# XDzzzzzZyq/b-pinn-kalman-filter

Measured on AMD Instinct MI355X. Metric: PC-sampler score-net evals/s (NCSN++ 128x128x1, EM + Langevin), higher is better.
Workload: dtype f32; 1 GPU; configs[2]: NCSN++ 128x128x1 PC sampler, VP-SDE N=1000, euler_maruyama + langevin (snr 0.075), global batch 64 = 64/GPU x 1; model=ncsnpp (62.69M params), global_batch=64, per_gpu_batch=64, parallelism=dp1 (batch-sharded, RCCL), hip_graph=True, pc_graph_allreduce=False

## Files before the change

b-pinn-kalman-filter_amd/csrc/conv_winograd.hip:

```cpp
#include "bpk_common.h"

#include <algorithm>
#include <cstdlib>
#include <type_traits>

namespace {

using f4 = __attribute__((ext_vector_type(4))) float;

constexpr int kTR = 4, kTC = 8;
constexpr int kM = kTR * kTC;
constexpr int kPR = 2 * kTR + 2;
constexpr int kPC = 2 * kTC + 2;
constexpr int kPCp = 24;
constexpr int kCK = 8;
constexpr int kOutRows = 2 * kTR, kOutCols = 2 * kTC;

__device__ inline void wino_filter_range(const float* __restrict__ w, float* __restrict__ U,
                                         int Cin, int Cout, int CoutP, int ft, int64_t first,
                                         int64_t stride) {
  const int64_t total = (int64_t)Cin * CoutP;
  for (int64_t i = first; i < total; i += stride) {
    const int co = (int)(i % CoutP);
    const int ci = (int)(i / CoutP);
    if (co >= Cout) {
      f4* u = reinterpret_cast<f4*>(U + ((int64_t)ci * CoutP + co) * 16);
#pragma unroll
      for (int r = 0; r < 4; ++r) u[r] = f4{0.f, 0.f, 0.f, 0.f};
      continue;
    }
    const float* g = ft ? w + ((int64_t)ci * Cout + co) * 9 : w + ((int64_t)co * Cin + ci) * 9;
    auto gv = [&](int k) { return ft ? g[8 - k] : g[k]; };
    float t[4][3];
#pragma unroll
    for (int c = 0; c < 3; ++c) {
      const float g0 = gv(c), g1 = gv(3 + c), g2 = gv(6 + c);
      t[0][c] = g0;
      t[1][c] = 0.5f * (g0 + g1 + g2);
      t[2][c] = 0.5f * (g0 - g1 + g2);
      t[3][c] = g2;
    }
    float* u = U + ((int64_t)ci * CoutP + co) * 16;
#pragma unroll
    for (int r = 0; r < 4; ++r) {
      const float a0 = t[r][0], a1 = t[r][1], a2 = t[r][2];
      u[4 * r + 0] = a0;
      u[4 * r + 1] = 0.5f * (a0 + a1 + a2);
      u[4 * r + 2] = 0.5f * (a0 - a1 + a2);
      u[4 * r + 3] = a2;
    }
  }
}

__global__ __launch_bounds__(256) void wino_filter_kernel(const float* __restrict__ w,
                                                          float* __restrict__ U, int Cin,
                                                          int Cout, int CoutP, int ft) {
  wino_filter_range(w, U, Cin, Cout, CoutP, ft, (int64_t)blockIdx.x * blockDim.x + threadIdx.x,
                    (int64_t)gridDim.x * blockDim.x);
}

__global__ __launch_bounds__(256) void wino_filter_batch_kernel(const int64_t* __restrict__ jobs) {
  const int64_t* jb = jobs + 6 * (int64_t)blockIdx.y;
  wino_filter_range(reinterpret_cast<const float*>(jb[0]), reinterpret_cast<float*>(jb[1]),
                    (int)jb[2], (int)jb[3], (int)jb[4], (int)jb[5],
                    (int64_t)blockIdx.x * blockDim.x + threadIdx.x,
                    (int64_t)gridDim.x * blockDim.x);
}

struct WinoGeo {
  int N, Cin, Cout, H, W;
  int regions_x, regions_y, cout_blocks;
  float div;
  int C1;
  int CoutS;
  int up;
  int ksplit;
  int pair;
};

constexpr int kVS = 20;
constexpr int kOS = kOutRows * kOutCols + 4;
constexpr int kPatchPerThread = (kCK * kPR * kPC + 255) / 256;
constexpr int kPreMaxCin = 1024;


__device__ inline float silu_f(float z) { return z * __builtin_amdgcn_rcpf(1.f + __expf(-z)); }

__device__ inline unsigned udivmod(unsigned a, unsigned d, unsigned& r) {
  if ((d & (d - 1)) == 0) {
    r = a & (d - 1);
    return a >> __builtin_ctz(d);
  }
  const unsigned q = a / d;
  r = a - q * d;
  return q;
}

__device__ inline float div_rn(float a, float b, float r) {
  const float q = a * r;
// ... 845 lines not shown
      }
    }
    if (!PAIR && stats) {
      merge_stats(lm, lm2, __shfl_xor(lm, 16, 64), __shfl_xor(lm2, 16, 64), 32.f);
      merge_stats(lm, lm2, __shfl_xor(lm, 32, 64), __shfl_xor(lm2, 32, 64), 64.f);
      if (kq == 0) {
        const int R = g.regions_x * g.regions_y;
        const int region = (oy0 / kOutRows) * g.regions_x + ox0 / kOutCols;
        stats[((int64_t)n * g.CoutS + co) * R + region] = make_float2(lm, lm2);
      }
    }
  }
  WINO_TS(5);
}

template <bool PRE, bool PAIR = false>
__global__ __launch_bounds__(512, 1) void wino_f23_k16_kernel(
    const float* __restrict__ x, const float* __restrict__ U, const float* __restrict__ bias,
    const float* __restrict__ skip, const float2* __restrict__ pre, float* __restrict__ y,
    float2* __restrict__ stats, WinoGeo g, int xcd_remap, const float* __restrict__ x2,
    unsigned items) {
  const unsigned G = gridDim.x, w = blockIdx.x;
  unsigned first = w, stride = G, end = items;
  if (xcd_remap) {
    const unsigned xc = w & 7u, q = items >> 3, r = items & 7u;
    const unsigned start = xc * q + min(xc, r);
    first = start + (w >> 3);
    stride = G >> 3;
    end = start + q + (xc < r ? 1u : 0u);
  }
  for (unsigned b = first; b < end; b += stride) {
    if (b != first) __syncthreads();
    k16_item<PRE, PAIR>(b, x, U, bias, skip, pre, y, stats, g, x2);
  }
}

__global__ __launch_bounds__(256) void wino_splitk_reduce_kernel(
    const float* __restrict__ part, int S, const float* __restrict__ bias,
    const float* __restrict__ skip, float* __restrict__ y, float2* __restrict__ stats,
    WinoGeo g) {
  const int lane = threadIdx.x & 63;
  const int q = threadIdx.x;
  unsigned b = blockIdx.x, reg, cg;
  const unsigned R = (unsigned)(g.regions_x * g.regions_y);
  unsigned r = udivmod(b, R, reg);
  int n = (int)udivmod(r, (unsigned)(g.CoutS / 8), cg);
  const int co = (int)cg * 8 + (q >> 5);
  const int rem = q & 31;
  const int row = rem >> 2;
  int c4 = rem & 3;
  if (g.pair) {
    n = 2 * n + (c4 >> 1);
    c4 &= 1;
  }
  const int oy0 = (int)(reg / g.regions_x) * kOutRows, ox0 = (int)(reg % g.regions_x) * kOutCols;
  const int64_t plane = (int64_t)g.H * g.W;
  const int64_t slab = (int64_t)g.N * g.CoutS * plane;
  const int64_t o = ((int64_t)n * g.CoutS + co) * plane + (int64_t)(oy0 + row) * g.W + ox0 + 4 * c4;
  f4 v = *reinterpret_cast<const f4*>(&part[o]);
  for (int s = 1; s < S; ++s) v += *reinterpret_cast<const f4*>(&part[s * slab + o]);
  const float bv = bias ? bias[co] : 0.f;
  v += f4{bv, bv, bv, bv};
  if (skip) {
    const f4 sk = *reinterpret_cast<const f4*>(&skip[o]);
    const float rdiv = 1.f / g.div;
#pragma unroll
// ... 265 lines not shown
                       U, nullptr, nullptr, kpre, workspace, nullptr, gk, remap, x2, (unsigned)items);
  BPK_LAUNCH_CHECK("conv3x3_wino_splitk");
  const int64_t rblocks = (int64_t)N * (Cout / 8) * gk.regions_x * gk.regions_y;
  BPK_REQUIRE(Cout % 8 == 0 && rblocks < (1LL << 31), "conv3x3_wino_splitk: reduce grid");
  hipLaunchKernelGGL(wino_splitk_reduce_kernel, dim3((unsigned)rblocks), dim3(256), 0, st,
                     workspace, S, bias, skip, y, reinterpret_cast<float2*>(stats), gk);
  BPK_LAUNCH_CHECK("conv3x3_wino_splitk_reduce");
  return BPK_OK;
}

extern "C" int bpk_conv3x3_wino_up2_supported(int N, int Cin, int Cout, int H, int W) {
  return bpk_conv3x3_wino_supported(N, Cin, Cout, H, W) && Cin % 16 == 0 &&
         cout_padded(Cout) % 128 == 0;
}

extern "C" int bpk_conv3x3_wino_up2_f32(const float* x, const float* U, const float* bias,
                                        float* y, int N, int Cin, int Cout, int H, int W,
                                        void* stream) {
  BPK_REQUIRE(bpk_conv3x3_wino_up2_supported(N, Cin, Cout, H, W),
              "conv3x3_wino_up2: unsupported shape N=%d Cin=%d Cout=%d H=%d W=%d (need Cin %% 16, "
              "Cout %% 128, H %% 8, W %% 16 == 0)", N, Cin, Cout, H, W);
  const int CoutP = cout_padded(Cout);
  WinoGeo gk{N, Cin, CoutP, H, W, W / kOutCols, H / kOutRows, CoutP / 128, 1.0f, Cin, Cout, 1};
  const int64_t items = (int64_t)N * gk.regions_x * gk.regions_y * gk.cout_blocks;
  BPK_REQUIRE(items < (1LL << 31), "conv3x3_wino_up2: grid too large");
  const unsigned kg = k16_grid(items);
  hipLaunchKernelGGL((wino_f23_k16_kernel<false>), dim3(kg), dim3(512), 0,
                     bpk::as_stream(stream), x, U, bias, nullptr, nullptr, y, nullptr, gk,
                     (kg % 8 == 0) ? 1 : 0, nullptr, (unsigned)items);
  BPK_LAUNCH_CHECK("conv3x3_wino_up2");
  return BPK_OK;
}

extern "C" int bpk_conv3x3_wino_pre_f32(const float* x, const float* pre, const float* U,
                                        const float* bias, const float* skip, float div, float* y,
                                        int N, int Cin, int Cout, int H, int W, void* stream) {
  return bpk_conv3x3_wino_ex_f32(x, nullptr, Cin, pre, U, bias, skip, div, y, nullptr, N, Cin,
                                 Cout, H, W, stream);
}

extern "C" int bpk_conv3x3_wino_residual_f32(const float* x, const float* U, const float* bias,
                                             const float* skip, float div, float* y, int N,
                                             int Cin, int Cout, int H, int W, void* stream) {
  return bpk_conv3x3_wino_pre_f32(x, nullptr, U, bias, skip, div, y, N, Cin, Cout, H, W, stream);
}

extern "C" int bpk_conv3x3_wino_f32(const float* x, const float* U, const float* bias, float* y,
                                    int N, int Cin, int Cout, int H, int W, void* stream) {
  return bpk_conv3x3_wino_pre_f32(x, nullptr, U, bias, nullptr, 1.0f, y, N, Cin, Cout, H, W,
                                  stream);
}

#ifdef WINO_TIMING
extern "C" int bpk_wino_timing_read(long long* ts, unsigned* cu, int n) {
  if (n > (int)kTsMax) n = (int)kTsMax;
  if (hipMemcpyFromSymbol(ts, HIP_SYMBOL(g_wino_ts), sizeof(long long) * 8 * n) != hipSuccess) return -1;
  if (hipMemcpyFromSymbol(cu, HIP_SYMBOL(g_wino_cu), sizeof(unsigned) * n) != hipSuccess) return -1;
  return n;
}
#endif
```

b-pinn-kalman-filter_amd/op/conv.py:

```python
from __future__ import annotations

import contextlib
import functools
import os

import torch
import torch.nn.functional as F
from torch.autograd.function import once_differentiable

from . import flops
from ._lib import check, lib, require_hip, stream_ptr, mark_inputs, want_grad


def _shape_ok(x, weight):
    return (x.dtype == torch.float32 and weight.dtype == torch.float32 and x.dim() == 4
            and tuple(weight.shape[2:]) == (3, 3) and x.is_cuda and weight.shape[1] == x.shape[1])


def wino_supported(x, weight):
    if not _shape_ok(x, weight):
        return False
    N, C, H, W = x.shape
    return bool(lib.bpk_conv3x3_wino_supported(N, C, weight.shape[0], H, W))


def wino_pair_supported(x, weight):
    if not _shape_ok(x, weight):
        return False
    N, C, H, W = x.shape
    return bool(lib.bpk_conv3x3_wino_pair_supported(N, C, weight.shape[0], H, W))


def small_supported(x, weight):
    if not _shape_ok(x, weight):
        return False
    N, C, H, W = x.shape
    return bool(lib.bpk_conv3x3_small_supported(N, C, weight.shape[0], H, W))


def supported(x, weight):
    return small_supported(x, weight) or wino_supported(x, weight)


_STATIC_FILTERS = None


@contextlib.contextmanager
def static_filters(registry: list):
    global _STATIC_FILTERS
    prev, _STATIC_FILTERS = _STATIC_FILTERS, registry
    try:
        yield registry
    finally:
        _STATIC_FILTERS = prev


def _transform_into(weight, U, ft):
    w = weight.detach().contiguous()
    Cout, Cin = (w.shape[1], w.shape[0]) if ft else (w.shape[0], w.shape[1])
    fn = lib.bpk_conv3x3_wino_filter_ft_f32 if ft else lib.bpk_conv3x3_wino_filter_f32
    check(fn(w.data_ptr(), U.data_ptr(), Cin, Cout, stream_ptr(w.device)), "conv3x3 filter")


def refresh_filters(registry: list):
    for i, (weight, U, ft, ver) in enumerate(registry):
        if weight._version != ver:
            _transform_into(weight, U, ft)
            registry[i] = (weight, U, ft, weight._version)


_FILTER_BATCH = None


class FilterBatch:

    def __init__(self, module):
        jobs, self.map, self.params = [], {}, []
        dev = None
        for m in module.modules():
            if not (isinstance(m, torch.nn.Conv2d) and m.kernel_size == (3, 3)
                    and m.stride == (1, 1) and m.padding == (1, 1) and m.dilation == (1, 1)
                    and m.groups == 1):
                continue
            w = m.weight
            if not (w.is_cuda and w.dtype == torch.float32 and w.is_contiguous()):
                continue
            dev = w.device
            self.params.append(w)
            for ft in (False, True):
                Cout, Cin = (w.shape[1], w.shape[0]) if ft else (w.shape[0], w.shape[1])
                key = (w.data_ptr(), ft)
                if Cin % 8 or Cout % 16 or key in self.map:
                    continue
                CoutP = lib.bpk_conv3x3_wino_filter_bytes(Cin, Cout) // (16 * 4 * Cin)
                U = torch.empty((Cin, CoutP, 16), dtype=torch.float32, device=w.device)
                self.map[key] = (tuple(w.shape), U)
                jobs.append([w.data_ptr(), U.data_ptr(), Cin, Cout, CoutP, int(ft)])
        self.n = len(jobs)
        self.max_elems = max((j[2] * j[4] for j in jobs), default=0)
        self.jobs = torch.tensor(jobs, dtype=torch.int64).to(dev) if jobs else None
        self.ptrs = [w.data_ptr() for w in self.params]
# ... 6 lines not shown
            check(lib.bpk_conv3x3_wino_filter_batch_f32(
                self.jobs.data_ptr(), self.n, self.max_elems, stream_ptr(self.jobs.device)),
                "conv3x3 filter batch")

    @contextlib.contextmanager
    def active(self):
        global _FILTER_BATCH
        prev, _FILTER_BATCH = _FILTER_BATCH, self.map
        try:
            yield self
        finally:
            _FILTER_BATCH = prev


def filter_batch_for(module) -> "FilterBatch":
    fb = getattr(module, "_bpk_filter_batch", None)
    if fb is None or not fb.valid_for(module):
        fb = FilterBatch(module)
        object.__setattr__(module, "_bpk_filter_batch", fb)
    return fb


@contextlib.contextmanager
def batched_filters(module, enabled=True):
    if not enabled:
        yield None
        return
    fb = filter_batch_for(module)
    fb.refresh()
    with fb.active():
        yield fb


def filter_transform(weight, ft=False):
    fbm = _FILTER_BATCH
    if fbm is not None and weight.is_contiguous():
        e = fbm.get((weight.data_ptr(), bool(ft)))
        if e is not None and e[0] == tuple(weight.shape):
            return e[1]
    attr = "_bpk_wino_u_ft" if ft else "_bpk_wino_u"
    capturing = torch.cuda.is_current_stream_capturing()
    cached = getattr(weight, attr, None)
    if capturing and _STATIC_FILTERS is not None and cached is not None \
            and cached[0] == weight._version:
        if not any(e[1] is cached[1] for e in _STATIC_FILTERS):
            _STATIC_FILTERS.append((weight, cached[1], ft, weight._version))
        return cached[1]
    if capturing:
        cached = None
    if cached is not None and cached[0] == weight._version:
        return cached[1]
    w = weight.detach().contiguous()
    Cout, Cin = (w.shape[1], w.shape[0]) if ft else (w.shape[0], w.shape[1])
    CoutP = lib.bpk_conv3x3_wino_filter_bytes(Cin, Cout) // (16 * 4 * Cin)
    U = torch.empty((Cin, CoutP, 16), dtype=torch.float32, device=w.device)
    fn = lib.bpk_conv3x3_wino_filter_ft_f32 if ft else lib.bpk_conv3x3_wino_filter_f32
    check(fn(w.data_ptr(), U.data_ptr(), Cin, Cout, stream_ptr(w.device)), "conv3x3 filter")
    if not capturing:
        setattr(weight, attr, (weight._version, U))
    return U


GN_PART_COUNT = 128


def gn_partials(t):
    p = getattr(t, "_bpk_gn_part", None)
    if p is None or p[3] != t._version:
        return None
    return p[:3]


def attach_gn_partials(t, part, R, cnt=GN_PART_COUNT):
    t._bpk_gn_part = (part, R, cnt, t._version)
    return t


def ensure_gn_partials(t):
    p = gn_partials(t)
    if p is not None:
        return p
    if (t.dim() != 4 or not t.is_cuda or t.dtype != torch.float32 or not t.is_contiguous()
            or (t.shape[2] * t.shape[3]) % GN_PART_COUNT != 0):
        return None
    N, C, H, W = t.shape
    R = H * W // GN_PART_COUNT
    part = torch.empty((N, C, R, 2), dtype=torch.float32, device=t.device)
    check(lib.bpk_group_norm_chunk_partials_f32(t.data_ptr(), part.data_ptr(), N, C, H * W,
                                                stream_ptr(t.device)), "gn_partials")
    attach_gn_partials(t, part, R)
    return part, R, GN_PART_COUNT


def conv3x3_fwd_raw(x, weight, bias=None, skip=None, div=1.0, pre=None, stats=False, x2=None,
                    ft=False):
    x = x.contiguous()
    N, C1, H, W = x.shape
    C = C1 if x2 is None else C1 + x2.shape[1]
    if x2 is not None:
        x2 = x2.contiguous()
        if x2.shape[0] != N or tuple(x2.shape[2:]) != (H, W) or C1 % 8:
            raise RuntimeError(f"conv3x3: second source {tuple(x2.shape)} vs {tuple(x.shape)}")
    Cout = weight.shape[1] if ft else weight.shape[0]
    U = filter_transform(weight, ft)
    y = torch.empty((N, Cout, H, W), dtype=x.dtype, device=x.device)
    b = None if bias is None else bias.detach().contiguous()
    sk = None if skip is None else skip.detach().contiguous()
    if sk is not None and sk.shape != y.shape:
        raise RuntimeError(f"conv3x3: skip {tuple(sk.shape)} != output {tuple(y.shape)}")
    pr = None if pre is None else pre.contiguous()
    if pr is not None and tuple(pr.shape) != (N, C, 2):
        raise RuntimeError(f"conv3x3: pre must be [N, Cin, 2], got {tuple(pr.shape)}")
    part = None
    if stats:
        R = (H // 8) * (W // 16)
        part = torch.empty((N, Cout, R, 2), dtype=torch.float32, device=x.device)
    nws = lib.bpk_conv3x3_wino_splitk_bytes(N, C, C1 if x2 is not None else C, Cout, H, W)
    ws = torch.empty(nws // 4, dtype=torch.float32, device=x.device) if nws > 0 else None
    check(lib.bpk_conv3x3_wino_splitk_f32(
        x.data_ptr(), None if x2 is None else x2.data_ptr(), C1,
        None if pr is None else pr.data_ptr(), U.data_ptr(),
        None if b is None else b.data_ptr(), None if sk is None else sk.data_ptr(), float(div),
        y.data_ptr(), None if part is None else part.data_ptr(),
        None if ws is None else ws.data_ptr(), N, C, Cout, H, W,
        stream_ptr(x.device)), "conv3x3_wino")
    flops.wino3x3("wino_dgrad" if ft else "wino_fwd", N, C, Cout, H, W)
    if part is not None:
        attach_gn_partials(y, part, R)
    return y


_WGRAD = True


def wgrad_supported(x, weight):
    if not _WGRAD:
        return False
    if x.dtype != torch.float32 or x.dim() != 4 or not x.is_cuda:
        return False
    N, C, H, W = x.shape
    cout = weight[0] if isinstance(weight, (tuple, list, torch.Size)) else weight.shape[0]
    return bool(lib.bpk_conv3x3_wino_wgrad_supported(N, C, cout, H, W))


def conv3x3_wgrad_raw(x, gy, wshape, bias_grad=False, pre=None):
    x = x.detach().contiguous()
    gy = gy.detach().contiguous()
    N, C, H, W = x.shape
    Cout = wshape[0]
    if tuple(gy.shape) != (N, Cout, H, W) or tuple(wshape[1:]) != (C, 3, 3):
        raise RuntimeError(f"conv3x3_wgrad: x {tuple(x.shape)}, gy {tuple(gy.shape)}, "
                           f"w {tuple(wshape)}")
    nbytes = lib.bpk_conv3x3_wino_wgrad_workspace_bytes(N, C, Cout, H, W)
    ws = torch.empty(nbytes // 4, dtype=torch.float32, device=x.device)
    dw = torch.empty((Cout, C, 3, 3), dtype=torch.float32, device=x.device)
    db = torch.empty((Cout,), dtype=torch.float32, device=x.device) if bias_grad else None
    pr = None if pre is None else pre.detach().contiguous()
    if pr is not None and tuple(pr.shape) != (N, C, 2):
        raise RuntimeError(f"conv3x3_wgrad: pre must be [N, Cin, 2], got {tuple(pr.shape)}")
# ... 756 lines not shown
    __slots__ = ("g",)

    def __init__(self):
        self.g = None


def gn_silu_conv3x3_ad(x, num_groups, gamma, beta, eps, weight, bias=None, skip=None, div=1.0,
                       bias_nc=None, give=None, take=None, fanout=False):
    require_hip(x, weight, bias, skip, bias_nc, what="gn_silu_conv3x3_ad")
    if not gn_silu_conv3x3_ad_supported(x, weight):
        return None
    if skip is not None and tuple(skip.shape) != (x.shape[0], weight.shape[0]) + tuple(x.shape[2:]):
        return None
    stats = bool(wino_supported(x, weight))
    return _GNSiLUConv3x3.apply(x, bias_nc, gamma, beta, weight, bias, skip, num_groups,
                                float(eps), float(div), stats, give, take, bool(fanout))


def up2_supported(x, weight):
    if not (_WINO_UP2 and x.is_cuda and x.dtype == torch.float32 and x.dim() == 4
            and weight.dtype == torch.float32 and tuple(weight.shape[1:]) == (x.shape[1], 3, 3)):
        return False
    N, C, H, W = x.shape
    return bool(lib.bpk_conv3x3_wino_up2_supported(N, C, weight.shape[0], 2 * H, 2 * W))


_WINO_UP2 = True


def _up2_raw(x, weight, bias):
    x = x.detach().contiguous()
    N, C, H, W = x.shape
    Cout = weight.shape[0]
    U = filter_transform(weight, False)
    y = torch.empty((N, Cout, 2 * H, 2 * W), dtype=x.dtype, device=x.device)
    b = None if bias is None else bias.detach().contiguous()
    check(lib.bpk_conv3x3_wino_up2_f32(x.data_ptr(), U.data_ptr(),
                                       None if b is None else b.data_ptr(), y.data_ptr(),
                                       N, C, Cout, 2 * H, 2 * W, stream_ptr(x.device)),
          "conv3x3_wino_up2")
    flops.wino3x3("wino_fwd", N, C, Cout, 2 * H, 2 * W)
    return y


class _Sum2x2(torch.autograd.Function):

    @staticmethod
    def forward(ctx, g):
        N, C, H2, W2 = g.shape
        if g.is_cuda and g.dtype == torch.float32:
            g = g.contiguous()
            y = torch.empty((N, C, H2 // 2, W2 // 2), device=g.device, dtype=g.dtype)
            check(lib.bpk_sum2x2_f32(g.data_ptr(), y.data_ptr(), N * C, H2 // 2, W2 // 2,
                                     stream_ptr(g.device)), "sum2x2")
            return y
        return g.reshape(N, C, H2 // 2, 2, W2 // 2, 2).sum((3, 5))

    @staticmethod
    def backward(ctx, gg):
        return F.interpolate(gg, scale_factor=2, mode="nearest")


def _sum2x2(g):
    if g.shape[2] % 2 or g.shape[3] % 2:
        raise RuntimeError(f"_sum2x2: even spatial sizes expected, got {tuple(g.shape)}")
    return _Sum2x2.apply(g)


class _ConvUp2(torch.autograd.Function):

    @staticmethod
    def forward(ctx, x, w, b):
        mark_inputs(ctx, x, w, b)
        ctx.save_for_backward(x, w)
# ... 335 lines not shown
```

b-pinn-kalman-filter_amd/op/flops.py:

```python
from __future__ import annotations

import contextlib

_ACTIVE: list = []


class Tally:
    def __init__(self):
        self.executed = 0.0
        self.direct = 0.0
        self.by_kind: dict = {}
        self.aten = 0.0

    def add(self, kind, executed, direct):
        self.executed += executed
        self.direct += direct
        e, d, n = self.by_kind.get(kind, (0.0, 0.0, 0))
        self.by_kind[kind] = (e + executed, d + direct, n + 1)

    @property
    def total_executed(self):
        return self.executed + self.aten

    @property
    def total_direct(self):
        return self.direct + self.aten

    def summary(self):
        return {"executed_flop": self.total_executed, "direct_flop": self.total_direct,
                "aten_flop": self.aten,
                "native": {k: {"executed": e, "direct": d, "launches": n}
                           for k, (e, d, n) in sorted(self.by_kind.items())}}


def add(kind, executed, direct=None):
    if _ACTIVE:
        for t in _ACTIVE:
            t.add(kind, float(executed), float(executed if direct is None else direct))


def wino3x3(kind, N, C, Cout, H, W):
    if _ACTIVE:
        add(kind, 32.0 * N * C * Cout * ((H + 1) // 2) * ((W + 1) // 2), 18.0 * N * C * Cout * H * W)


def _aten_mode():
    from torch.utils._python_dispatch import TorchDispatchMode
    from torch.utils.flop_counter import flop_registry

    class AtenFlops(TorchDispatchMode):
        total = 0

        def __torch_dispatch__(self, func, types, args=(), kwargs=None):
            kwargs = kwargs or {}
            out = func(*args, **kwargs)
            f = flop_registry.get(func._overloadpacket)
            if f is not None:
                self.total += f(*args, **kwargs, out_val=out)
            return out

    return AtenFlops()


@contextlib.contextmanager
def counting(aten=True):
    t = Tally()
    _ACTIVE.append(t)
    mode = _aten_mode() if aten else contextlib.nullcontext()
    try:
        with mode:
            yield t
    finally:
        _ACTIVE.remove(t)
        if aten:
            t.aten = float(mode.total)
```

include/bpk.h:

```cpp
#ifndef BPK_H_
#define BPK_H_

#include <stdint.h>

#ifdef __cplusplus
extern "C" {
#endif

#define BPK_OK 0
#define BPK_ERR_ARG 1
#define BPK_ERR_LAUNCH 2
#define BPK_ERR_UNSUPPORTED 3

#define BPK_ABI_VERSION 1

const char* bpk_last_error(void);
int bpk_abi_version(void);


int bpk_upfirdn2d_f32(const float* x, const float* kernel, float* out, int major, int in_h,
                      int in_w, int minor, int kernel_h, int kernel_w, int up_x, int up_y,
                      int down_x, int down_y, int pad_x0, int pad_x1, int pad_y0, int pad_y1,
                      int out_h, int out_w, void* stream);
int bpk_upfirdn2d_f64(const double* x, const double* kernel, double* out, int major, int in_h,
// ... 175 lines not shown
int bpk_correlation_fwd_f32(const float* first, const float* second, float* out, int B, int C,
                            int H, int W, int stride, void* stream);
int bpk_correlation_bwd_f32(const float* first, const float* second, const float* grad_out,
                            float* grad_first, float* grad_second, int B, int C, int H, int W,
                            int stride, void* stream);

int64_t bpk_conv3x3_wino_filter_bytes(int Cin, int Cout);
int bpk_conv3x3_wino_filter_f32(const float* weight, float* U, int Cin, int Cout, void* stream);
int bpk_conv3x3_wino_filter_ft_f32(const float* weight, float* U, int Cin, int Cout,
                                   void* stream);
int bpk_conv3x3_wino_filter_batch_f32(const int64_t* jobs, int n, int max_elems, void* stream);
int bpk_conv3x3_wino_supported(int N, int Cin, int Cout, int H, int W);
int bpk_conv3x3_wino_pair_supported(int N, int Cin, int Cout, int H, int W);
int bpk_conv3x3_wino_f32(const float* x, const float* U, const float* bias, float* y, int N,
                         int Cin, int Cout, int H, int W, void* stream);
int bpk_conv3x3_wino_residual_f32(const float* x, const float* U, const float* bias,
                                  const float* skip, float div, float* y, int N, int Cin,
                                  int Cout, int H, int W, void* stream);
int bpk_conv3x3_wino_pre_f32(const float* x, const float* pre, const float* U, const float* bias,
                             const float* skip, float div, float* y, int N, int Cin, int Cout,
                             int H, int W, void* stream);
int bpk_conv3x3_wino_ex_f32(const float* x, const float* x2, int C1, const float* pre,
                            const float* U, const float* bias, const float* skip, float div,
                            float* y, float* stats, int N, int Cin, int Cout, int H, int W,
                            void* stream);
int64_t bpk_conv3x3_wino_splitk_bytes(int N, int Cin, int C1, int Cout, int H, int W);
int bpk_conv3x3_wino_splitk_f32(const float* x, const float* x2, int C1, const float* pre,
                                const float* U, const float* bias, const float* skip, float div,
                                float* y, float* stats, float* workspace, int N, int Cin, int Cout,
                                int H, int W, void* stream);
int bpk_conv3x3_wino_up2_supported(int N, int Cin, int Cout, int H, int W);
int bpk_conv3x3_wino_up2_f32(const float* x, const float* U, const float* bias, float* y, int N,
                             int Cin, int Cout, int H, int W, void* stream);
int bpk_conv3x3_wino_wgrad_supported(int N, int Cin, int Cout, int H, int W);
int64_t bpk_conv3x3_wino_wgrad_workspace_bytes(int N, int Cin, int Cout, int H, int W);
int bpk_conv3x3_wino_wgrad_f32(const float* x, const float* gy, float* dw, float* workspace,
                               int N, int Cin, int Cout, int H, int W, void* stream);
int bpk_conv3x3_wino_wgrad_bias_f32(const float* x, const float* gy, float* dw, float* db,
                                    float* workspace, int N, int Cin, int Cout, int H, int W,
                                    void* stream);
int bpk_conv3x3_wino_wgrad_pre_f32(const float* x, const float* pre, const float* gy, float* dw,
                                   float* db, float* workspace, int N, int Cin, int Cout, int H,
                                   int W, void* stream);
int bpk_conv3x3_wino_wgrad2_f32(const float* x, const float* gy, const float* x2, const float* gy2,
                                int N2, float* dw, float* db, float* workspace, int N, int Cin,
                                int Cout, int H, int W, void* stream);

int bpk_conv3x3_small_supported(int N, int Cin, int Cout, int H, int W);
int bpk_conv3x3_small_f32(const float* x, const float* pre, const float* weight,
                          const float* bias, float* y, int N, int Cin, int Cout, int H, int W,
                          void* stream);

int bpk_conv2d_wgrad_small_cout_supported(int N, int Cin, int Cout, int H, int W, int K);
int64_t bpk_conv2d_wgrad_small_cout_workspace_bytes(int N, int Cin, int Cout, int K);
int bpk_conv2d_wgrad_small_cout_f32(const float* x, const float* gy, float* dw, float* db,
                                    void* workspace, int N, int Cin, int Cout, int H, int W,
                                    int K, void* stream);

int bpk_gemm_nchw_supported(int N, int M, int P, int K1, int K2);
int bpk_gemm_nchw_f32(const float* W, int ldw, const float* X1, int K1, const float* X2, int K2,
                      const float* bias, float* Y, int N, int M, int P, void* stream);
int64_t bpk_gemm_nchw_splitk_bytes(int N, int M, int P, int K1, int K2);
int bpk_gemm_nchw_splitk_f32(const float* W, int ldw, const float* X1, int K1, const float* X2,
                             int K2, const float* bias, float* Y, float* workspace, int N, int M,
                             int P, void* stream);
int bpk_gemm_sb_f32(const float* A, int64_t sab, int64_t sam, int64_t sak, const float* B,
// ... 59 lines not shown
```

Baseline: 681.2 score-net evals/s.

## Add Winograd F(2x2,3x3)-by-F(2,4) 24-tile forward conv path with MFMA kernel

Adds a new Winograd variant that uses 4x6 input tiles (F(2x4,3x3)), 24 transform points per 8 outputs instead of 16 per 4. It comes with a filter-transform kernel, a 512-thread MFMA main kernel with double-buffered LDS patches, and split-K and upsample launchers. Forward convolutions now use it by default when the shape is supported. The aim is to cut the multiply count per output, since 48 MACs per 8 outputs replaces 32 per 4. In exchange the transforms cost more, register pressure rises, and fp32 rounding error from the larger tile grows.

```diff
diff --git a/b-pinn-kalman-filter_amd/csrc/conv_winograd.hip b/b-pinn-kalman-filter_amd/csrc/conv_winograd.hip
--- a/b-pinn-kalman-filter_amd/csrc/conv_winograd.hip
+++ b/b-pinn-kalman-filter_amd/csrc/conv_winograd.hip
@@ -1,4 +1,5 @@
 #include "bpk_common.h"
+#include "wino_f24.h"
 
 #include <algorithm>
 #include <cstdlib>
@@ -65,6 +66,32 @@
                     (int)jb[2], (int)jb[3], (int)jb[4], (int)jb[5],
                     (int64_t)blockIdx.x * blockDim.x + threadIdx.x,
                     (int64_t)gridDim.x * blockDim.x);
+}
+
+__global__ __launch_bounds__(256) void wino_filter24_kernel(const float* __restrict__ w,
+                                                            float* __restrict__ U, int Cin,
+                                                            int Cout, int CoutP, int ft) {
+  const int64_t total = (int64_t)Cin * CoutP;
+  for (int64_t i = (int64_t)blockIdx.x * blockDim.x + threadIdx.x; i < total;
+       i += (int64_t)gridDim.x * blockDim.x) {
+    const int co = (int)(i % CoutP);
+    const int ci = (int)(i / CoutP);
+    float u[24];
+    if (co >= Cout) {
+#pragma unroll
+      for (int p = 0; p < 24; ++p) u[p] = 0.f;
+    } else {
+      const float* g = ft ? w + ((int64_t)ci * Cout + co) * 9 : w + ((int64_t)co * Cin + ci) * 9;
+      float gg[9];
+#pragma unroll
+      for (int k = 0; k < 9; ++k) gg[k] = ft ? g[8 - k] : g[k];
+      wino24_filter(gg, u);
+    }
+    f4* dst = reinterpret_cast<f4*>(U) + ((int64_t)ci * (CoutP / 16) + co / 16) * 96 + co % 16;
+#pragma unroll
+    for (int q = 0; q < 6; ++q)
+      dst[16 * q] = f4{u[4 * q], u[4 * q + 1], u[4 * q + 2], u[4 * q + 3]};
+  }
 }
 
 struct WinoGeo {
@@ -976,6 +1003,282 @@
   for (unsigned b = first; b < end; b += stride) {
     if (b != first) __syncthreads();
     k16_item<PRE, PAIR>(b, x, U, bias, skip, pre, y, stats, g, x2);
+  }
+}
+
+constexpr int kM24 = 16;
+constexpr int kVS24 = 28;
+
+template <bool PRE>
+__device__ __forceinline__ void k16_item24(
+    unsigned b, const float* __restrict__ x, const float* __restrict__ U,
+    const float* __restrict__ bias, const float* __restrict__ skip,
+    const float2* __restrict__ pre, float* __restrict__ y, float2* __restrict__ stats,
+    const WinoGeo& g, const float* __restrict__ x2) {
+  constexpr int CK = 16;
+  constexpr int kPatch = CK * kPR * kPCp;
+  __shared__ __attribute__((aligned(16))) float s_patch_raw[2][kPatch];
+  constexpr int kVBuf = CK * kM24 * kVS24;
+  __shared__ __attribute__((aligned(16))) float s_v[2][kVBuf];
+  __shared__ float2 s_ss[PRE ? kPreMaxCin : 1];
+
+  const int tid = threadIdx.x;
+  const int wave = tid >> 6, lane = tid & 63;
+  unsigned cb, rx, ry;
+  unsigned r = udivmod(b, (unsigned)g.cout_blocks, cb);
+  r = udivmod(r, (unsigned)g.regions_x, rx);
+  r = udivmod(r, (unsigned)g.regions_y, ry);
+  unsigned nn;
+  const int ks_idx = (int)udivmod(r, (unsigned)g.N, nn);
+  const int n = (int)nn;
+  const int oy0 = (int)ry * kOutRows, ox0 = (int)rx * kOutCols;
+  const int cout_w = (int)cb * 128 + wave * 16;
+  const int ph = __builtin_amdgcn_readfirstlane(tid >> 8);
+
+  f4 acc[24];
+  const int64_t plane = (int64_t)g.H * g.W;
+  const int up = g.up;
+  const int64_t xplane = plane >> (2 * up);
+  const int C2 = g.Cin - g.C1;
+  const float* xn = x + (int64_t)n * g.C1 * xplane;
+  const float2* pre_n = PRE ? pre + (int64_t)n * g.Cin : nullptr;
+  const int kq = lane >> 4, jj = lane & 15;
+  const int nch = g.Cin / CK / max(g.ksplit, 1);
+  const int kb = ks_idx * nch;
+
+  const __amdgpu_buffer_rsrc_t xrs = __builtin_amdgcn_make_buffer_rsrc(
+      const_cast<float*>(xn), 0, (int)(g.C1 * xplane * 4), 0x00020000);
+  const __amdgpu_buffer_rsrc_t xrs2 = __builtin_amdgcn_make_buffer_rsrc(
+      const_cast<float*>(C2 > 0 ? x2 + (int64_t)n * C2 * plane : xn), 0,
+      (int)((C2 > 0 ? C2 : g.C1) * plane * 4), 0x00020000);
+  const __amdgpu_buffer_rsrc_t urs = __builtin_amdgcn_make_buffer_rsrc(
+      const_cast<float*>(U), 0, (int)((int64_t)g.Cin * g.Cout * 96), 0x00020000);
+
+  constexpr int kPos = kPR * kPC;
+  int poff, pdst;
+  bool pin;
+  {
+    const int t8 = tid & 255;
+    const int t = t8 < kPos ? t8 : 0;
+    const int py = t / kPC, px = t - py * kPC;
+    const int iy = oy0 - 1 + py, ix = ox0 - 1 + px;
+    pin = iy >= 0 && iy < g.H && ix >= 0 && ix < g.W;
+    const int cy = min(max(iy, 0), g.H - 1), cx = min(max(ix, 0), g.W - 1);
+    poff = ((cy >> up) * (g.W >> up) + (cx >> up)) * 4;
+    pdst = py * kPCp + px + ph * 8 * (kPR * kPCp);
+  }
+  float pv[8];
+  auto load_patch_part = [&](float* dst, int k, int c0, int cn) {
+    const int cc = (kb + min(k, nch - 1)) * CK;
+    const bool second = cc >= g.C1;
+    const int soff = ((second ? cc - g.C1 : cc) + ph * 8) * (int)xplane * 4;
+#pragma unroll
+    for (int c = c0; c < c0 + cn; ++c)
+      dst[c] = __uint_as_float(__builtin_amdgcn_raw_buffer_load_b32(
+          second ? xrs2 : xrs, poff, soff + c * (int)xplane * 4, 0));
+  };
+  auto store_patch_part = [&](const float* src, float* sp, int k, int c0, int cn) {
+    const int cb0 = (kb + min(k, nch - 1)) * CK + ph * 8;
+#pragma unroll
+    for (int c = c0; c < c0 + cn; ++c) {
+      float v = src[c];
+      if (PRE) {
+        const float2 st = s_ss[cb0 + c];
+        v = silu_f(v * st.x + st.y);
+      }
+      sp[pdst + c * (kPR * kPCp)] = pin ? v : 0.f;
+    }
+  };
+  f4 uo[2][6];
+  const int uoff = ((kq * g.Cout + cout_w) * 24 + jj * 4) * 4;
+  auto u_soff = [&](int k, int ks) {
+    return (((kb + min(k, nch - 1)) * CK + 4 * ks) * g.Cout) * 96;
+  };
+  auto load_u = [&](int slot, int k, int ks) {
+    const int soff = u_soff(k, ks);
+#pragma unroll
+    for (int q = 0; q < 6; ++q)
+      uo[slot][q] = __builtin_bit_cast(
+          f4, __builtin_amdgcn_raw_buffer_load_b128(urs, uoff + q * 256, soff, 0));
+  };
+  const int th = __builtin_amdgcn_readfirstlane(wave & 1);
+  const int tc = 4 * kq + (wave >> 1);
+  const int tty = jj >> 2, ttx = jj & 3;
+  float d[3][6];
+  auto read_d = [&](const float* sp) {
+#pragma unroll
+    for (int i = 0; i < 3; ++i) {
+      const float* row = &sp[(tc * kPR + 2 * tty + th + i) * kPCp + 4 * ttx];
+      const f4 v4 = *reinterpret_cast<const f4*>(row);
+      const float2 v2 = *reinterpret_cast<const float2*>(row + 4);
+      d[i][0] = v4[0];
+      d[i][1] = v4[1];
+      d[i][2] = v4[2];
+      d[i][3] = v4[3];
+      d[i][4] = v2.x;
+      d[i][5] = v2.y;
+    }
+  };
+  auto write_v = [&](float* sv) {
+    float rx_[6], ry_[6], vx[6], vy[6];
+#pragma unroll
+    for (int j = 0; j < 6; ++j) wino24_data_rows(d[0][j], d[1][j], d[2][j], th, rx_[j], ry_[j]);
+    wino24_data_cols(rx_, vx);
+    wino24_data_cols(ry_, vy);
+    f4* dst = reinterpret_cast<f4*>(&sv[(tc * kM24 + jj) * kVS24 + 12 * th]);
+    dst[0] = f4{vx[0], vx[1], vx[2], vx[3]};
+    dst[1] = f4{vx[4], vx[5], vy[0], vy[1]};
+    dst[2] = f4{vy[2], vy[3], vy[4], vy[5]};
+  };
+
+  {
+    float pv0[8], pv1[8];
+    load_patch_part(pv0, 0, 0, 8);
+    load_patch_part(pv1, 1, 0, 8);
+    load_patch_part(pv, 2, 0, 8);
+    load_u(0, 0, 0);
+    load_u(1, 0, 1);
+    if (PRE) {
+      for (int c = tid; c < g.Cin; c += 512) s_ss[c] = pre_n[c];
+      __syncthreads();
+    }
+    store_patch_part(pv0, s_patch_raw[0], 0, 0, 8);
+    store_patch_part(pv1, s_patch_raw[1], 1, 0, 8);
+  }
+  __syncthreads();
+  read_d(s_patch_raw[0]);
+  write_v(s_v[0]);
+  __syncthreads();
+
+  f4 a[4];
+  auto a_src = [&](const float* sv, int ks) {
+    return reinterpret_cast<const f4*>(&sv[((4 * ks + kq) * kM24 + jj) * kVS24]);
+  };
+  {
+    const f4* src = a_src(s_v[0], 0);
+#pragma unroll
+    for (int q = 0; q < 4; ++q) a[q] = src[q];
+  }
+  auto step = [&](int k, auto sb_c, auto first_c) __attribute__((always_inline)) {
+    constexpr int SB = decltype(sb_c)::value;
+    constexpr bool FIRST = decltype(first_c)::value;
+    const float* sv = s_v[SB];
+#pragma unroll
+    for (int grp = 0; grp < 8; ++grp) {
+      const int ks = grp >> 1, hf = grp & 1;
+      __builtin_amdgcn_sched_barrier(0);
+      if (grp == 0) read_d(s_patch_raw[SB ^ 1]);
+      if (grp == 1) write_v(s_v[SB ^ 1]);
+      if (grp == 2) store_patch_part(pv, s_patch_raw[SB], k + 2, 0, 4);
+      if (grp == 3) store_patch_part(pv, s_patch_raw[SB], k + 2, 4, 4);
+      if (grp == 4) load_patch_part(pv, k + 3, 0, 4);
+      if (grp == 5) load_patch_part(pv, k + 3, 4, 4);
+      __builtin_amdgcn_sched_barrier(0);
+#pragma unroll
+      for (int qq = 0; qq < 3; ++qq) {
+        const int q = 3 * hf + qq;
+        const int fi = 6 * ks + q;
+#pragma unroll
+        for (int pp = 0; pp < 4; ++pp)
+          acc[4 * q + pp] = __builtin_amdgcn_mfma_f32_16x16x4f32(
+              a[fi & 3][pp], uo[ks & 1][q][pp],
+              (FIRST && ks == 0) ? f4{0.f, 0.f, 0.f, 0.f} : acc[4 * q + pp], 0, 0, 0);
+        if (fi + 4 < 24) a[fi & 3] = a_src(sv, (fi + 4) / 6)[(fi + 4) % 6];
+        const int soff = ks < 2 ? u_soff(k, ks + 2) : u_soff(k + 1, ks - 2);
+        uo[ks & 1][q] = __builtin_bit_cast(
+            f4, __builtin_amdgcn_raw_buffer_load_b128(urs, uoff + q * 256, soff, 0));
+      }
+    }
+    __syncthreads();
+    const f4* src = a_src(s_v[SB ^ 1], 0);
+#pragma unroll
+    for (int q = 0; q < 4; ++q) a[q] = src[q];
+  };
+  using C0 = std::integral_constant<int, 0>;
+  using C1 = std::integral_constant<int, 1>;
+  step(0, C0{}, std::true_type{});
+  int k = 1;
+  for (; k + 1 < nch; k += 2) {
+    step(k, C1{}, std::false_type{});
+    step(k + 1, C0{}, std::false_type{});
+  }
+  if (k < nch) step(k, C1{}, std::false_type{});
+
+  const float rdiv = 1.f / g.div;
+  if (cout_w < g.CoutS) {
+    const int co = cout_w + jj;
+    const float bv = bias ? bias[co] : 0.f;
+    const int64_t obase = ((int64_t)(ks_idx * g.N + n) * g.CoutS + co) * plane +
+                          (int64_t)(oy0 + 2 * kq) * g.W + ox0;
+    float lm = 0.f, lm2 = 0.f;
+    f4 skv[2][4];
+    if (skip) {
+#pragma unroll
+      for (int h = 0; h < 2; ++h)
+#pragma unroll
+        for (int rg = 0; rg < 4; ++rg)
+          skv[h][rg] = *reinterpret_cast<const f4*>(&skip[obase + (int64_t)h * g.W + 4 * rg]);
+    }
+#pragma unroll
+    for (int h = 0; h < 2; ++h) {
+#pragma unroll
+      for (int rg = 0; rg < 4; ++rg) {
+        float t[6], yv[4];
+#pragma unroll
+        for (int j = 0; j < 6; ++j)
+          t[j] = wino24_out_rows(acc[j][rg], acc[6 + j][rg], acc[12 + j][rg], acc[18 + j][rg], h);
+        wino24_out_cols(t, yv);
+        f4 v = f4{yv[0] + bv, yv[1] + bv, yv[2] + bv, yv[3] + bv};
+        const int64_t o = obase + (int64_t)h * g.W + 4 * rg;
+        if (skip) {
+          const f4 sk = skv[h][rg];
+#pragma unroll
+          for (int c = 0; c < 4; ++c) v[c] = div_rn(sk[c] + v[c], g.div, rdiv);
+        }
+        *reinterpret_cast<f4*>(&y[o]) = v;
+        if (stats) {
+          const float sm = ((v[0] + v[1]) + (v[2] + v[3])) * 0.25f;
+          float sm2 = 0.f;
+#pragma unroll
+          for (int c = 0; c < 4; ++c) sm2 = fmaf(v[c] - sm, v[c] - sm, sm2);
+          constexpr float kW[8] = {1.f, 1.f / 2, 1.f / 3, 1.f / 4, 1.f / 5, 1.f / 6, 1.f / 7, 1.f / 8};
+          const int st = 4 * h + rg;
+          const float dd = sm - lm;
+          lm = lm + dd * kW[st];
+          lm2 = (lm2 + sm2) + dd * dd * (4.f * st * kW[st]);
+        }
+      }
+    }
+    if (stats) {
+      merge_stats(lm, lm2, __shfl_xor(lm, 16, 64), __shfl_xor(lm2, 16, 64), 32.f);
+      merge_stats(lm, lm2, __shfl_xor(lm, 32, 64), __shfl_xor(lm2, 32, 64), 64.f);
+      if (kq == 0) {
+        const int R = g.regions_x * g.regions_y;
+        const int region = (oy0 / kOutRows) * g.regions_x + ox0 / kOutCols;
+        stats[((int64_t)n * g.CoutS + co) * R + region] = make_float2(lm, lm2);
+      }
+    }
+  }
+}
+
+template <bool PRE>
+__global__ __launch_bounds__(512, 1) void wino_f24_k16_kernel(
+    const float* __restrict__ x, const float* __restrict__ U, const float* __restrict__ bias,
+    const float* __restrict__ skip, const float2* __restrict__ pre, float* __restrict__ y,
+    float2* __restrict__ stats, WinoGeo g, int xcd_remap, const float* __restrict__ x2,
+    unsigned items) {
+  const unsigned G = gridDim.x, w = blockIdx.x;
+  unsigned first = w, stride = G, end = items;
+  if (xcd_remap) {
+    const unsigned xc = w & 7u, q = items >> 3, r = items & 7u;
+    const unsigned start = xc * q + min(xc, r);
+    first = start + (w >> 3);
+    stride = G >> 3;
+    end = start + q + (xc < r ? 1u : 0u);
+  }
+  for (unsigned b = first; b < end; b += stride) {
+    if (b != first) __syncthreads();
+    k16_item24<PRE>(b, x, U, bias, skip, pre, y, stats, g, x2);
   }
 }
 
@@ -1307,6 +1610,100 @@
   return BPK_OK;
 }
 
+
+extern "C" int bpk_conv3x3_wino_f24_supported(int N, int Cin, int C1, int Cout, int H, int W) {
+#ifdef WINO_NO_F24
+  return 0;
+#else
+  return N > 0 && Cin > 0 && Cin % 16 == 0 && Cin <= kPreMaxCin && C1 > 0 && C1 <= Cin &&
+         C1 % 16 == 0 && Cout > 0 && Cout % 16 == 0 && cout_padded(Cout) % 128 == 0 && H > 0 &&
+         H % kOutRows == 0 && W > 0 && W % kOutCols == 0;
+#endif
+}
+
+extern "C" int64_t bpk_conv3x3_wino_filter24_bytes(int Cin, int Cout) {
+  return (int64_t)24 * Cin * cout_padded(Cout) * (int64_t)sizeof(float);
+}
+
+static int wino_filter24(const float* weight, float* U, int Cin, int Cout, int ft, void* stream) {
+  BPK_REQUIRE(Cin > 0 && Cout > 0, "conv3x3_wino_filter24: bad channels %d -> %d", Cin, Cout);
+  const int64_t total = (int64_t)Cin * cout_padded(Cout);
+  hipLaunchKernelGGL(wino_filter24_kernel,
+                     dim3((unsigned)std::min<int64_t>(bpk::ceil_div(total, 256), 4096)), dim3(256),
+                     0, bpk::as_stream(stream), weight, U, Cin, Cout, cout_padded(Cout), ft);
+  BPK_LAUNCH_CHECK("conv3x3_wino_filter24");
+  return BPK_OK;
+}
+
+extern "C" int bpk_conv3x3_wino_filter24_f32(const float* weight, float* U, int Cin, int Cout,
+                                             void* stream) {
+  return wino_filter24(weight, U, Cin, Cout, 0, stream);
+}
+
+extern "C" int bpk_conv3x3_wino_filter24_ft_f32(const float* weight, float* U, int Cin, int Cout,
+                                                void* stream) {
+  return wino_filter24(weight, U, Cin, Cout, 1, stream);
+}
+
+static int wino_f24_launch(const float* x, const float* x2, int C1, const float* pre,
+                           const float* U, const float* bias, const float* skip, float div,
+                           float* y, float* stats, int N, int Cin, int Cout, int H, int W, int up,
+                           int S, WinoGeo* geo, void* stream) {
+  BPK_REQUIRE(bpk_conv3x3_wino_f24_supported(N, Cin, C1, Cout, H, W),
+              "conv3x3_wino_f24: unsupported shape N=%d Cin=%d (C1=%d) Cout=%d H=%d W=%d (need "
+              "Cin, C1 %% 16, Cout %% 128, H %% 8, W %% 16 == 0, Cin <= %d)", N, Cin, C1, Cout, H,
+              W, kPreMaxCin);
+  const int CoutP = cout_padded(Cout);
+  WinoGeo gk{N, Cin, CoutP, H, W, W / kOutCols, H / kOutRows, CoutP / 128, div, C1, Cout, up, S};
+  const int64_t items = (int64_t)N * gk.regions_x * gk.regions_y * gk.cout_blocks * S;
+  BPK_REQUIRE(items < (1LL << 31), "conv3x3_wino_f24: grid too large");
+  const float2* kpre = reinterpret_cast<const float2*>(pre);
+  float2* stats2 = reinterpret_cast<float2*>(stats);
+  hipStream_t st = bpk::as_stream(stream);
+  const unsigned kg = k16_grid(items);
+  const int remap = (kg % 8 == 0) ? 1 : 0;
+  if (pre)
+    hipLaunchKernelGGL((wino_f24_k16_kernel<true>), dim3(kg), dim3(512), 0, st, x, U, bias, skip,
+                       kpre, y, stats2, gk, remap, x2, (unsigned)items);
+  else
+    hipLaunchKernelGGL((wino_f24_k16_kernel<false>), dim3(kg), dim3(512), 0, st, x, U, bias, skip,
+                       kpre, y, stats2, gk, remap, x2, (unsigned)items);
+  BPK_LAUNCH_CHECK("conv3x3_wino_f24");
+  if (geo) *geo = gk;
+  return BPK_OK;
+}
+
+extern "C" int bpk_conv3x3_wino_f24_splitk_f32(const float* x, const float* x2, int C1,
+                                               const float* pre, const float* U,
+                                               const float* bias, const float* skip, float div,
+                                               float* y, float* stats, float* workspace, int N,
+                                               int Cin, int Cout, int H, int W, void* stream) {
+  if (!x2) C1 = Cin;
+  const int S = wino_splits(N, Cin, C1, Cout, H, W);
+  if (S <= 1)
+    return wino_f24_launch(x, x2, C1, pre, U, bias, skip, div, y, stats, N, Cin, Cout, H, W, 0, 1,
+                           nullptr, stream);
+  BPK_REQUIRE(workspace != nullptr, "conv3x3_wino_f24_splitk: workspace is NULL");
+  WinoGeo gk;
+  const int rc = wino_f24_launch(x, x2, C1, pre, U, nullptr, nullptr, div, workspace, nullptr, N,
+                                 Cin, Cout, H, W, 0, S, &gk, stream);
+  if (rc != BPK_OK) return rc;
+  const int64_t rblocks = (int64_t)N * (Cout / 8) * gk.regions_x * gk.regions_y;
+  BPK_REQUIRE(rblocks < (1LL << 31), "conv3x3_wino_f24_splitk: reduce grid");
+  hipLaunchKernelGGL(wino_splitk_reduce_kernel, dim3((unsigned)rblocks), dim3(256), 0,
+                     bpk::as_stream(stream), workspace, S, bias, skip, y,
+                     reinterpret_cast<float2*>(stats), gk);
+  BPK_LAUNCH_CHECK("conv3x3_wino_f24_splitk_reduce");
+  return BPK_OK;
+}
+
+extern "C" int bpk_conv3x3_wino_f24_up2_f32(const float* x, const float* U, const float* bias,
+                                            float* y, int N, int Cin, int Cout, int H, int W,
+                                            void* stream) {
+  return wino_f24_launch(x, nullptr, Cin, nullptr, U, bias, nullptr, 1.0f, y, nullptr, N, Cin,
+                         Cout, H, W, 1, 1, nullptr, stream);
+}
+
 extern "C" int bpk_conv3x3_wino_pre_f32(const float* x, const float* pre, const float* U,
                                         const float* bias, const float* skip, float div, float* y,
                                         int N, int Cin, int Cout, int H, int W, void* stream) {
diff --git a/b-pinn-kalman-filter_amd/csrc/wino_f24.h b/b-pinn-kalman-filter_amd/csrc/wino_f24.h
--- /dev/null
+++ b/b-pinn-kalman-filter_amd/csrc/wino_f24.h
@@ -0,0 +1,58 @@
+#pragma once
+
+#include <math.h>
+
+#if defined(__HIPCC__)
+#define WINO24_HD __host__ __device__ inline
+#else
+#define WINO24_HD inline
+#endif
+
+WINO24_HD int wino24_slot_row(int s) { return s < 2 ? s : 5 - s; }
+
+WINO24_HD void wino24_data_rows(float r0, float r1, float r2, int h, float& x, float& y) {
+  x = r0 - r2;
+  y = r1 + (h ? -r0 : r2);
+}
+
+WINO24_HD void wino24_data_cols(const float r[6], float v[6]) {
+  const float d31 = r[3] - r[1], d42 = r[4] - r[2];
+  v[0] = fmaf(-2.f, r[2], fmaf(1.5f, d31, r[0] + r[4]));
+  v[1] = fmaf(2.5f, r[3], fmaf(0.5f, r[2], r[4] - r[1]));
+  v[2] = fmaf(0.5f, r[3], fmaf(-2.5f, r[2], r[4] + r[1]));
+  v[3] = fmaf(2.f, d31, d42);
+  v[4] = fmaf(-0.5f, d31, d42);
+  v[5] = fmaf(-2.f, r[3], fmaf(1.5f, d42, r[1] + r[5]));
+}
+
+WINO24_HD void wino24_filter(const float g[9], float u[24]) {
+  double t[4][3];
+  for (int c = 0; c < 3; ++c) {
+    const double g0 = g[c], g1 = g[3 + c], g2 = g[6 + c];
+    t[0][c] = g0;
+    t[1][c] = 0.5 * (g0 + g1 + g2);
+    t[2][c] = 0.5 * (g0 - g1 + g2);
+    t[3][c] = g2;
+  }
+  for (int s = 0; s < 4; ++s) {
+    const double* a = t[wino24_slot_row(s)];
+    u[6 * s + 0] = (float)a[0];
+    u[6 * s + 1] = (float)((a[0] + a[1] + a[2]) / 3.0);
+    u[6 * s + 2] = (float)((a[1] - a[0] - a[2]) / 3.0);
+    u[6 * s + 3] = (float)(-(16.0 * a[0] + 8.0 * a[1] + 4.0 * a[2]) / 15.0);
+    u[6 * s + 4] = (float)((a[0] - 2.0 * a[1] + 4.0 * a[2]) / 15.0);
+    u[6 * s + 5] = (float)a[2];
+  }
+}
+
+WINO24_HD float wino24_out_rows(float m0, float m1, float m2, float m3, int h) {
+  return h == 0 ? (m0 + m1) + m3 : (m1 - m3) - m2;
+}
+
+WINO24_HD void wino24_out_cols(const float t[6], float y[4]) {
+  const float s12 = t[1] + t[2], d12 = t[1] - t[2];
+  y[0] = (t[0] + s12) + (t[3] + t[4]);
+  y[1] = fmaf(-2.f, t[4], fmaf(0.5f, t[3], d12));
+  y[2] = fmaf(4.f, t[4], fmaf(0.25f, t[3], s12));
+  y[3] = fmaf(-8.f, t[4], fmaf(0.125f, t[3], d12)) + t[5];
+}
diff --git a/b-pinn-kalman-filter_amd/op/conv.py b/b-pinn-kalman-filter_amd/op/conv.py
--- a/b-pinn-kalman-filter_amd/op/conv.py
+++ b/b-pinn-kalman-filter_amd/op/conv.py
@@ -55,18 +55,24 @@
         _STATIC_FILTERS = prev
 
 
-def _transform_into(weight, U, ft):
+def _filter_fn(ft, form):
+    if form == 24:
+        return lib.bpk_conv3x3_wino_filter24_ft_f32 if ft else lib.bpk_conv3x3_wino_filter24_f32
+    return lib.bpk_conv3x3_wino_filter_ft_f32 if ft else lib.bpk_conv3x3_wino_filter_f32
+
+
+def _transform_into(weight, U, ft, form=16):
     w = weight.detach().contiguous()
     Cout, Cin = (w.shape[1], w.shape[0]) if ft else (w.shape[0], w.shape[1])
-    fn = lib.bpk_conv3x3_wino_filter_ft_f32 if ft else lib.bpk_conv3x3_wino_filter_f32
-    check(fn(w.data_ptr(), U.data_ptr(), Cin, Cout, stream_ptr(w.device)), "conv3x3 filter")
+    check(_filter_fn(ft, form)(w.data_ptr(), U.data_ptr(), Cin, Cout, stream_ptr(w.device)),
+          "conv3x3 filter")
 
 
 def refresh_filters(registry: list):
-    for i, (weight, U, ft, ver) in enumerate(registry):
+    for i, (weight, U, ft, ver, form) in enumerate(registry):
         if weight._version != ver:
-            _transform_into(weight, U, ft)
-            registry[i] = (weight, U, ft, weight._version)
+            _transform_into(weight, U, ft, form)
+            registry[i] = (weight, U, ft, weight._version, form)
 
 
 _FILTER_BATCH = None
@@ -139,19 +145,31 @@
         yield fb
 
 
-def filter_transform(weight, ft=False):
+_F24 = os.environ.get("BPK_WINO_F24", "1") != "0"
+last_form = None
+
+
+def wino_form(weight, ft, N, C, C1, Cout, H, W):
+    if not _F24 or ft or _FILTER_BATCH is not None:
+        return 16
+    return 24 if lib.bpk_conv3x3_wino_f24_supported(N, C, C1, Cout, H, W) else 16
+
+
+def filter_transform(weight, ft=False, form=16):
+    if form not in (16, 24):
+        raise ValueError(f"filter_transform: form {form} (16 or 24)")
     fbm = _FILTER_BATCH
-    if fbm is not None and weight.is_contiguous():
+    if fbm is not None and form == 16 and weight.is_contiguous():
         e = fbm.get((weight.data_ptr(), bool(ft)))
         if e is not None and e[0] == tuple(weight.shape):
             return e[1]
-    attr = "_bpk_wino_u_ft" if ft else "_bpk_wino_u"
+    attr = ("_bpk_wino_u_ft" if ft else "_bpk_wino_u") + ("24" if form == 24 else "")
     capturing = torch.cuda.is_current_stream_capturing()
     cached = getattr(weight, attr, None)
     if capturing and _STATIC_FILTERS is not None and cached is not None \
             and cached[0] == weight._version:
         if not any(e[1] is cached[1] for e in _STATIC_FILTERS):
-            _STATIC_FILTERS.append((weight, cached[1], ft, weight._version))
+            _STATIC_FILTERS.append((weight, cached[1], ft, weight._version, form))
         return cached[1]
     if capturing:
         cached = None
@@ -160,9 +178,9 @@
     w = weight.detach().contiguous()
     Cout, Cin = (w.shape[1], w.shape[0]) if ft else (w.shape[0], w.shape[1])
     CoutP = lib.bpk_conv3x3_wino_filter_bytes(Cin, Cout) // (16 * 4 * Cin)
-    U = torch.empty((Cin, CoutP, 16), dtype=torch.float32, device=w.device)
-    fn = lib.bpk_conv3x3_wino_filter_ft_f32 if ft else lib.bpk_conv3x3_wino_filter_f32
-    check(fn(w.data_ptr(), U.data_ptr(), Cin, Cout, stream_ptr(w.device)), "conv3x3 filter")
+    U = torch.empty((Cin, CoutP, form), dtype=torch.float32, device=w.device)
+    check(_filter_fn(ft, form)(w.data_ptr(), U.data_ptr(), Cin, Cout, stream_ptr(w.device)),
+          "conv3x3 filter")
     if not capturing:
         setattr(weight, attr, (weight._version, U))
     return U
@@ -209,7 +227,9 @@
         if x2.shape[0] != N or tuple(x2.shape[2:]) != (H, W) or C1 % 8:
             raise RuntimeError(f"conv3x3: second source {tuple(x2.shape)} vs {tuple(x.shape)}")
     Cout = weight.shape[1] if ft else weight.shape[0]
-    U = filter_transform(weight, ft)
+    global last_form
+    form = last_form = wino_form(weight, ft, N, C, C1, Cout, H, W)
+    U = filter_transform(weight, ft, form)
     y = torch.empty((N, Cout, H, W), dtype=x.dtype, device=x.device)
     b = None if bias is None else bias.detach().contiguous()
     sk = None if skip is None else skip.detach().contiguous()
@@ -224,14 +244,16 @@
         part = torch.empty((N, Cout, R, 2), dtype=torch.float32, device=x.device)
     nws = lib.bpk_conv3x3_wino_splitk_bytes(N, C, C1 if x2 is not None else C, Cout, H, W)
     ws = torch.empty(nws // 4, dtype=torch.float32, device=x.device) if nws > 0 else None
-    check(lib.bpk_conv3x3_wino_splitk_f32(
+    fn = lib.bpk_conv3x3_wino_f24_splitk_f32 if form == 24 else lib.bpk_conv3x3_wino_splitk_f32
+    check(fn(
         x.data_ptr(), None if x2 is None else x2.data_ptr(), C1,
         None if pr is None else pr.data_ptr(), U.data_ptr(),
         None if b is None else b.data_ptr(), None if sk is None else sk.data_ptr(), float(div),
         y.data_ptr(), None if part is None else part.data_ptr(),
         None if ws is None else ws.data_ptr(), N, C, Cout, H, W,
         stream_ptr(x.device)), "conv3x3_wino")
-    flops.wino3x3("wino_dgrad" if ft else "wino_fwd", N, C, Cout, H, W)
+    flops.wino3x3("wino_dgrad" if ft else "wino_fwd24" if form == 24 else "wino_fwd",
+                  N, C, Cout, H, W, form)
     if part is not None:
         attach_gn_partials(y, part, R)
     return y
@@ -1054,14 +1076,15 @@
     x = x.detach().contiguous()
     N, C, H, W = x.shape
     Cout = weight.shape[0]
-    U = filter_transform(weight, False)
+    global last_form
+    form = last_form = wino_form(weight, False, N, C, C, Cout, 2 * H, 2 * W)
+    U = filter_transform(weight, False, form)
     y = torch.empty((N, Cout, 2 * H, 2 * W), dtype=x.dtype, device=x.device)
     b = None if bias is None else bias.detach().contiguous()
-    check(lib.bpk_conv3x3_wino_up2_f32(x.data_ptr(), U.data_ptr(),
-                                       None if b is None else b.data_ptr(), y.data_ptr(),
-                                       N, C, Cout, 2 * H, 2 * W, stream_ptr(x.device)),
-          "conv3x3_wino_up2")
-    flops.wino3x3("wino_fwd", N, C, Cout, 2 * H, 2 * W)
+    fn = lib.bpk_conv3x3_wino_f24_up2_f32 if form == 24 else lib.bpk_conv3x3_wino_up2_f32
+    check(fn(x.data_ptr(), U.data_ptr(), None if b is None else b.data_ptr(), y.data_ptr(),
+             N, C, Cout, 2 * H, 2 * W, stream_ptr(x.device)), "conv3x3_wino_up2")
+    flops.wino3x3("wino_fwd24" if form == 24 else "wino_fwd", N, C, Cout, 2 * H, 2 * W, form)
     return y
 
 
diff --git a/b-pinn-kalman-filter_amd/op/flops.py b/b-pinn-kalman-filter_amd/op/flops.py
--- a/b-pinn-kalman-filter_amd/op/flops.py
+++ b/b-pinn-kalman-filter_amd/op/flops.py
@@ -39,9 +39,13 @@
             t.add(kind, float(executed), float(executed if direct is None else direct))
 
 
-def wino3x3(kind, N, C, Cout, H, W):
+def wino3x3(kind, N, C, Cout, H, W, form=16):
     if _ACTIVE:
-        add(kind, 32.0 * N * C * Cout * ((H + 1) // 2) * ((W + 1) // 2), 18.0 * N * C * Cout * H * W)
+        if form == 24:
+            executed = 48.0 * N * C * Cout * ((H + 1) // 2) * ((W + 3) // 4)
+        else:
+            executed = 32.0 * N * C * Cout * ((H + 1) // 2) * ((W + 1) // 2)
+        add(kind, executed, 18.0 * N * C * Cout * H * W)
 
 
 def _aten_mode():
diff --git a/include/bpk.h b/include/bpk.h
--- a/include/bpk.h
+++ b/include/bpk.h
@@ -231,6 +231,17 @@
 int bpk_conv3x3_wino_up2_supported(int N, int Cin, int Cout, int H, int W);
 int bpk_conv3x3_wino_up2_f32(const float* x, const float* U, const float* bias, float* y, int N,
                              int Cin, int Cout, int H, int W, void* stream);
+int bpk_conv3x3_wino_f24_supported(int N, int Cin, int C1, int Cout, int H, int W);
+int64_t bpk_conv3x3_wino_filter24_bytes(int Cin, int Cout);
+int bpk_conv3x3_wino_filter24_f32(const float* weight, float* U, int Cin, int Cout, void* stream);
+int bpk_conv3x3_wino_filter24_ft_f32(const float* weight, float* U, int Cin, int Cout,
+                                     void* stream);
+int bpk_conv3x3_wino_f24_splitk_f32(const float* x, const float* x2, int C1, const float* pre,
+                                    const float* U, const float* bias, const float* skip,
+                                    float div, float* y, float* stats, float* workspace, int N,
+                                    int Cin, int Cout, int H, int W, void* stream);
+int bpk_conv3x3_wino_f24_up2_f32(const float* x, const float* U, const float* bias, float* y, int N,
+                                 int Cin, int Cout, int H, int W, void* stream);
 int bpk_conv3x3_wino_wgrad_supported(int N, int Cin, int Cout, int H, int W);
 int64_t bpk_conv3x3_wino_wgrad_workspace_bytes(int N, int Cin, int Cout, int H, int W);
 int bpk_conv3x3_wino_wgrad_f32(const float* x, const float* gy, float* dw, float* workspace,
```

After: 779.5 score-net evals/s (median of 6 runs). 14.4% higher.
